# jzhoulab/orca

Hardware: AMD Instinct MI355X
Metric: Mb of sequence encoded+decoded per second (32Mb H1-ESC-shaped model, both strands, 6 levels) (higher is better)
Workload: dtype f16x2 | Encoder Conv1d stages 1-7: f16x2 = fp32 emulated as 2 x fp16 split operands, 3 MFMA products, fp32 accumulate (22 significant operand bits); Decoder / Decoder_1m Conv2d: f16x2 = fp32 emulated as 2 x fp16 split operands, 3 MFMA products, fp32 accumulate (22 significant operand bits); Encoder2; 1 GPU; H1-ESC 32Mb model forward, single random 32Mb sequence, fp32-class (f16x2 split operands on the 16-bit matrix cores, see dtype; parity vs the reference's fp32 in `parity` with --full), both strands (genomepredict-equivalent, 1 model): Encoder+Encoder2+6 Decoder+Decoder_1m per strand; sequence_bp=32000000, strands=2, levels=6, weights=synthetic seed 0, input=1 byte/base packed sequence in HBM, both strands read from it, parallelism=single GPU

## Files before the change

orca_amd/csrc/conv2d_dblock.h:

```cpp
#pragma once
#include "conv2d_m16.h"

struct DBlockArgs {
  f32x4* cur;
  const void* w[4];
  const float* bias[4];
  long bs;
  int H, W, dil;
  unsigned* flag;
};

#ifndef DBLOCK_STORE_WT
#define DBLOCK_STORE_WT 0
#endif
__device__ __forceinline__ void db_store_unit(u32x4_t* p, const u32x4_t& v) {
#if DBLOCK_STORE_WT
  m16_store_unit(p, v);
#else
  *p = v;
#endif
}

template <int NS, int DT, int ABL = 0>
__global__ __launch_bounds__(512, NS == 1 ? 4 : 2) void conv2d_dblock_kernel(DBlockArgs a) {
  constexpr int WNS = DT == 1 ? 2 : 1;
  constexpr int NT = 512, PXW = 256 + 16;
  constexpr int AU = NS * 8 * PXW, BU = NS * 4 * PXW;
  constexpr int WP = NS * 9 * 2 * 32;
  constexpr int NPIECE = 16;
  constexpr int WIT = (WP + NT - 1) / NT;
  static_assert(NS * 8 * 256 / NT == 4 * NS, "gather: NS DMA instructions per thread and K-chunk of the first layer (the same for every wave)");
  constexpr int EXTRA = (WP - (WIT - 1) * NT + 63) / 64;
  __shared__ f32x4 smem[AU + BU + 3 * WP + 48];
  f32x4* const As = smem;
  f32x4* const Bs = smem + AU;
  f32x4* const Ws = smem + AU + BU;
  float* const bias_s = reinterpret_cast<float*>(smem + AU + BU + 3 * WP);

  const int tid = threadIdx.x, lane = tid & 63;
  const int wave = __builtin_amdgcn_readfirstlane(tid >> 6);
  const int l31 = lane & 31, g = lane >> 5;
  const int d = a.dil, H = a.H, W = a.W;
  const int ld = 31 - __builtin_clz(d);
  const int lS = 8 - ld, S = 1 << lS;
  const int lG = 2 * ld - 8, G = 1 << lG;
  f32x4* const cur = a.cur + (long)blockIdx.y * a.bs;

  int bx = (int)blockIdx.x;
  if (!(ABL & 64)) {
    const int xcd = bx & 7, t = bx >> 3;
    if (G == 1) { const int run = xcd * 4 + (t >> 3); bx = (run >> 1) * 16 + (run & 1) * 8 + (t & 7); }
    else if (G == 4) { const int pair = xcd * 16 + (t >> 1); bx = pair * 2 + (t & 1); }
  }
  auto pix = [&](int p, int& row, int& col, int& r, int& c) {
    const int sid = (bx << lG) + (p >> (2 * lS)), q = p & ((1 << (2 * lS)) - 1);
    r = q >> lS; c = q & (S - 1);
    row = (sid >> ld) + (r << ld);
    col = (sid & (d - 1)) + (c << ld);
  };
  {
    const int sid0 = bx << lG;
    if ((sid0 >> ld) >= H || (sid0 & (d - 1)) >= W) return;
  }

  if (tid < NS * 8 * 16) As[(tid >> 4) * PXW + 256 + (tid & 15)] = (f32x4)(0.f);
  if (tid >= 256 && tid < 256 + NS * 4 * 16) Bs[((tid - 256) >> 4) * PXW + 256 + (tid & 15)] = (f32x4)(0.f);
  __syncthreads();
  if (wave == 0 && lane < 48) {
    const float* src = lane < 8 ? a.bias[0] + 4 * lane : (lane < 24 ? a.bias[1] + 4 * (lane - 8) : (lane < 32 ? a.bias[2] + 4 * (lane - 24) : a.bias[3] + 4 * (lane - 32)));
    p16_glds16(reinterpret_cast<const f32x4*>(src), smem + AU + BU + 3 * WP);
  }

  auto piece_src = [&](int i, int u) -> const f32x4* {
    const int L = i >> 2, j = i & 3;
    const bool wide = L & 1;
    const int k = wide ? (j & 1) : j, h = wide ? (j >> 1) : 0, cout = wide ? 64 : 32;
    const int grp = u >> 5, co = u & 31;
    return reinterpret_cast<const f32x4*>(a.w[L]) + ((long)k * (WNS * 9 * 2) + grp) * cout + h * 32 + co;
  };
  auto issue_piece = [&](int i) {
    f32x4* dst = Ws + (i % 3) * WP;
#pragma unroll
    for (int it = 0; it < WIT; ++it) {
      const int u = tid + it * NT;
      if (u < WP) p16_glds16(piece_src(i, u), dst + it * NT + wave * 64);
    }
  };
  {
    int row, col, r_, c_;
    pix(tid & 255, row, col, r_, c_);
    const bool ok = row < H && col < W;
    const long off = ok ? (long)row * M16_PX + col : 255;
#pragma unroll
    for (int k = 0; k < 4; ++k) {
#pragma unroll
      for (int s_ = 0; s_ < NS; ++s_) {
        const int plane = s_ * 8 + 2 * k + (wave >> 2);
        if (!(ABL & 4)) p16_glds16(cur + m16_plane(plane & 7, s_, NS, H) + off, As + plane * PXW + (wave & 3) * 64);
      }
      if (k < 3) issue_piece(k);
    }
  }

  const int p = wave * 32 + l31;
  int prow, pcol, pr, pc;
  pix(p, prow, pcol, pr, pc);
  const bool pvalid = prow < H && pcol < W;
  const long poff = (long)prow * M16_PX + pcol;
  unsigned nb16[9];
#pragma unroll
  for (int t = 0; t < 9; ++t) {
    const int dy = t / 3 - 1, dx = t % 3 - 1;
    const bool in = (unsigned)(pr + dy) < (unsigned)S && (unsigned)(pc + dx) < (unsigned)S;
    nb16[t] = (in ? (unsigned)(p + dy * S + dx) : 256u + ((unsigned)(p + dy * S + dx) & 15u)) * 16u;
  }

  f32x16 acc[2];
  int piece = 0;
  const unsigned as_lds = p16_lds_addr(As), bs_lds = p16_lds_addr(Bs), ws_lds = p16_lds_addr(Ws + g * 32 + l31);
#define DB_READ(buf_, t_)                                                                                         \
  _Pragma("unroll") for (int s = 0; s < NS; ++s) {                                                                \
    xv[buf_][s] = p16_lds_read16(xrow + nb16[t_], s * XG * PXW * 16);                                             \
    wv[buf_][s] = p16_lds_read16(wrow, ((s * 9 + (t_)) * 2) * 32 * 16);                                           \
  }
#define DB_LAYER(XLDS, XG_, WIDE)                                                                                 \
  {                                                                                                               \
    constexpr int XG = XG_;                                                                                       \
    _Pragma("unroll") for (int j = 0; j < 4; ++j, ++piece) {                                                      \
      constexpr bool wide_ = WIDE;                                                                                \
      const int k = wide_ ? (j & 1) : j;                                                                          \
      const int h = wide_ ? (j >> 1) : 0;                                                                         \
       \
       \
      if (piece == 0) {                                                                                           \
        if (wave < EXTRA) asm volatile("s_waitcnt vmcnt(%0)" ::"n"(3 * NS + 2 * WIT) : "memory");                \
        else asm volatile("s_waitcnt vmcnt(%0)" ::"n"(3 * NS + 2 * (WIT - 1)) : "memory");                       \
      } else if (piece == 1) {                                                                                    \
        if (wave < EXTRA) asm volatile("s_waitcnt vmcnt(%0)" ::"n"(2 * NS + WIT) : "memory");                    \
        else asm volatile("s_waitcnt vmcnt(%0)" ::"n"(2 * NS + WIT - 1) : "memory");                             \
      } else if (piece == 2) {                                                                                    \
        if (wave < EXTRA) asm volatile("s_waitcnt vmcnt(%0)" ::"n"(NS + WIT) : "memory");                        \
        else asm volatile("s_waitcnt vmcnt(%0)" ::"n"(NS + WIT - 1) : "memory");                                 \
      } else if (piece + 1 < NPIECE) {                                                                            \
        if (wave < EXTRA) asm volatile("s_waitcnt vmcnt(%0)" ::"n"(WIT) : "memory");                             \
        else asm volatile("s_waitcnt vmcnt(%0)" ::"n"(WIT - 1) : "memory");                                      \
      } else asm volatile("s_waitcnt vmcnt(0)" ::: "memory");                                                     \
       \
       \
       \
      if (!(ABL & 16) || j == 0) asm volatile("s_waitcnt lgkmcnt(0)\n\ts_barrier" ::: "memory");                                   \
      if (piece >= 1 && piece + 2 < NPIECE && !(ABL & 2)) issue_piece(piece + 2);    \
      const unsigned wrow = ws_lds + (unsigned)((piece % 3) * WP * 16);                                           \
      const unsigned xrow = (XLDS) + (unsigned)((2 * k + g) * PXW * 16);                                          \
      f16x8 xv[2][NS], wv[2][NS];                                                                                 \
      DB_READ(0, 0);                                                                                              \
      _Pragma("unroll") for (int t = 0; t < 9; ++t) {                                                             \
        const int fb = t & 1;                                                                                     \
        if (t + 1 < 9) { if (!(ABL & 8)) { DB_READ(fb ^ 1, t + 1); m16_wait<2 * NS, NS>(xv[fb], wv[fb]); } }      \
        else m16_wait<0, NS>(xv[fb], wv[fb]);                                                                     \
        typedef typename Op16<DT>::vec V_;                                                                        \
        if constexpr ((ABL & 1) != 0) { asm volatile("" ::"v"(xv[fb][0]), "v"(wv[fb][0])); } else                \
        if constexpr (NS == 2) {                                                                                  \
          acc[h] = Op16<DT>::mfma(__builtin_bit_cast(V_, wv[fb][0]), __builtin_bit_cast(V_, xv[fb][NS - 1]), acc[h]); \
          acc[h] = Op16<DT>::mfma(__builtin_bit_cast(V_, wv[fb][NS - 1]), __builtin_bit_cast(V_, xv[fb][0]), acc[h]); \
        }                                                                                                         \
        if constexpr ((ABL & 1) == 0) acc[h] = Op16<DT>::mfma(__builtin_bit_cast(V_, wv[fb][0]), __builtin_bit_cast(V_, xv[fb][0]), acc[h]); \
        __builtin_amdgcn_sched_barrier(0);                                                                        \
      }                                                                                                           \
    }                                                                                                             \
  }
  bool overflow = false;
  auto put = [&](f32x4* Xs, int XG, int oct, f32x4 v) {
    if (!pvalid) v = (f32x4)(0.f);
    u32x2 sp[NS];
    split4<NS, DT>(v, sp, overflow);
#pragma unroll
    for (int s = 0; s < NS; ++s) *reinterpret_cast<u32x2*>(reinterpret_cast<char*>(Xs + (s * XG + oct) * PXW + p) + 8 * g) = sp[s];
  };
  auto get_A = [&](int oct) -> f32x4 {
    float f[4] = {0.f, 0.f, 0.f, 0.f};
#pragma unroll
    for (int s = 0; s < NS; ++s) {
      const u32x2 u = *reinterpret_cast<const u32x2*>(reinterpret_cast<const char*>(As + (s * 8 + oct) * PXW + p) + 8 * g);
      float a0, a1, a2, a3;
      m16_pair<DT>(u.x, a0, a1);
      m16_pair<DT>(u.y, a2, a3);
      f[0] += a0; f[1] += a1; f[2] += a2; f[3] += a3;
    }
    f32x4 r;
    r.x = f[0]; r.y = f[1]; r.z = f[2]; r.w = f[3];
    return r;
  };
  auto acc4 = [&](int h, int q, int boff, bool relu) -> f32x4 {
    const f32x4 b = *reinterpret_cast<const f32x4*>(bias_s + boff + 8 * q + 4 * g);
    f32x4 v;
    v.x = acc[h][4 * q + 0] + b.x; v.y = acc[h][4 * q + 1] + b.y; v.z = acc[h][4 * q + 2] + b.z; v.w = acc[h][4 * q + 3] + b.w;
    if (relu) { v.x = p16_vmax(v.x, 0.f); v.y = p16_vmax(v.y, 0.f); v.z = p16_vmax(v.z, 0.f); v.w = p16_vmax(v.w, 0.f); }
    return v;
  };
  auto zero_acc = [&]() {
#pragma unroll
    for (int h = 0; h < 2; ++h)
#pragma unroll
      for (int r = 0; r < 16; ++r) acc[h][r] = 0.f;
  };

  zero_acc();
  DB_LAYER(as_lds, 8, false);
#pragma unroll
  for (int q = 0; q < 4; ++q) put(Bs, 4, q, acc4(0, q, 0, false));
  zero_acc();
  DB_LAYER(bs_lds, 4, true);
#pragma unroll
  for (int h = 0; h < 2; ++h)
#pragma unroll
    for (int q = 0; q < 4; ++q) put(As, 8, h * 4 + q, acc4(h, q, 32 + h * 32, false) + get_A(h * 4 + q));
  zero_acc();
  DB_LAYER(as_lds, 8, false);
#pragma unroll
  for (int q = 0; q < 4; ++q) put(Bs, 4, q, acc4(0, q, 96, true));
  zero_acc();
  DB_LAYER(bs_lds, 4, true);
#undef DB_LAYER
#undef DB_READ
  float vmax = 0.f;
  if constexpr (NS == 2) {
#pragma unroll
    for (int h = 0; h < 2; ++h)
#pragma unroll
      for (int q = 0; q < 4; ++q) {
        const f32x4 v = acc4(h, q, 128 + h * 32, true) + get_A(h * 4 + q);
        vmax = p16_vmax3_abs(p16_vmax3_abs(vmax, v.x, v.y), v.z, v.w);
        unsigned h0_, h1_, l0_, l1_;
        p16_split_hl(v, h0_, h1_, l0_, l1_);
        p16_swap32(h0_, l0_);
        p16_swap32(h1_, l1_);
        u32x4_t unit_;
        unit_.x = h0_; unit_.y = h1_; unit_.z = l0_; unit_.w = l1_;
        if (pvalid) db_store_unit(reinterpret_cast<u32x4_t*>(cur) + m16_plane(h * 4 + q, g, NS, H) + poff, unit_);
      }
    if (pvalid && vmax > 65504.f) overflow = true;
  } else {
#pragma unroll
    for (int h = 0; h < 2; ++h)
#pragma unroll
      for (int qp = 0; qp < 2; ++qp) {
        const f32x4 v0 = acc4(h, 2 * qp, 128 + h * 32, true) + get_A(h * 4 + 2 * qp);
        const f32x4 v1 = acc4(h, 2 * qp + 1, 128 + h * 32, true) + get_A(h * 4 + 2 * qp + 1);
        if (DT == 1) vmax = p16_vmax3_abs(p16_vmax3_abs(p16_vmax3_abs(p16_vmax3_abs(vmax, v0.x, v0.y), v0.z, v0.w), v1.x, v1.y), v1.z, v1.w);
        unsigned a0_ = m16_pk2<DT>(v0.x, v0.y), a1_ = m16_pk2<DT>(v0.z, v0.w), b0_ = m16_pk2<DT>(v1.x, v1.y), b1_ = m16_pk2<DT>(v1.z, v1.w);
        p16_swap32(a0_, b0_);
        p16_swap32(a1_, b1_);
        u32x4_t unit_;
        unit_.x = a0_; unit_.y = a1_; unit_.z = b0_; unit_.w = b1_;
        if (pvalid) db_store_unit(reinterpret_cast<u32x4_t*>(cur) + m16_plane(h * 4 + 2 * qp + g, 0, NS, H) + poff, unit_);
      }
    if (DT == 1 && pvalid && vmax > 65504.f) overflow = true;
  }
  if (DT == 1 && overflow && a.flag) *a.flag = 1u;
}
```

orca_amd/csrc/orca_decoder.hip:

```cpp
#include "orca_internal.h"

#include "conv2d_m16.h"
#include "conv2d_m16q.h"
#include "conv2d_dblock.h"
#include "misc_kernels.h"
#include "coarsegrain.h"

int launch_conv2d(orca_ctx* ctx, const ConvLayer& L, const float* x, long x_bs, float* y, long y_bs,
                         const float* r, long r_bs, int B, int n, int relu) {
  if (L.ksize != 3) return fail(ORCA_EINVAL, "launch_conv2d on a non-3x3 layer");
  Conv2dArgs a;
  a.x = x; a.w = L.d_w; a.bias = L.d_bias; a.y = y; a.r = r;
  a.x_bs = x_bs; a.y_bs = y_bs; a.r_bs = r_bs; a.H = n; a.W = n; a.dil = L.dil; a.nchunks = L.nchunks; a.relu = relu;
  dim3 grid((unsigned)n, (unsigned)B);
  if (L.cout == 64) hipLaunchKernelGGL((conv2d_3x3_kernel<64>), grid, dim3(512), 0, ctx->stream, a);
  else hipLaunchKernelGGL((conv2d_3x3_kernel<32>), grid, dim3(512), 0, ctx->stream, a);
  LAUNCHCHECK("conv2d_3x3_kernel");
  return ORCA_OK;
}

int launch_conv2d_m16(orca_ctx* ctx, const ConvLayer& L, const f32x4* x, long x_bs, int x_oct, f32x4* y, long y_bs, int y_oct,
                             const f32x4* r, long r_bs, int B, int n, int relu, int mode, int chunk0, int nchunks_,
                             const float* tab, long tab_bs) {
  const bool bf16 = mode == 1;
// ... 88 lines not shown
  ORCA_TRY(ws_ensure(ctx, need));
  auto take = [&](size_t units) { return reinterpret_cast<f32x4*>(ws_take(ctx, units * 4)); };
  float* const TAB0 = is1m ? nullptr : ws_take(ctx, B * tabsz);
  f32x4* const IN0 = take(B * szIN);
  f32x4* const A0 = take(B * szA);
  f32x4* const Bf0 = take(B * sz64);
  f32x4* const Cf0 = take(B * sz64);
  f32x4* const Df0 = take(B * sz64);
  f32x4* const T0 = take(B * sz32);
  auto run = [&](int b0, int nb) -> int {
    f32x4* IN = IN0 + b0 * szIN;
    f32x4* A = A0 + b0 * szA;
    f32x4* Bf = Bf0 + b0 * sz64;
    f32x4* Cf = Cf0 + b0 * sz64;
    f32x4* Df = Df0 + b0 * sz64;
    f32x4* T = T0 + b0 * sz32;
    hipStream_t s = ctx->stream;
    float* TAB = is1m ? nullptr : TAB0 + b0 * tabsz;
    auto emit = [&](const f32x4* buf, size_t bs) -> int {
      for (int b = 0; b < nb; ++b)
        hipLaunchKernelGGL((m16_to_nchw_kernel<NS, DT>), dim3((unsigned)n), dim3(ORCA_LDW), 0, s, buf + b * bs, probe->channels, n,
                           probe->out + (size_t)(b0 + b) * probe->channels * n * n);
      LAUNCHCHECK("m16_to_nchw_kernel");
      return ORCA_OK;
    };
#define PROBE(k, buf, bs) \
  if (probe && probe->stage == (k)) return emit(buf, bs)
    for (int c0 = 0; c0 < nb; c0 += 8) {
      const int nc = nb - c0 < 8 ? nb - c0 : 8;
      M16HeadArgs ha{};
      for (int b = 0; b < nc; ++b) { ha.x[b] = x.at(b0 + c0 + b); ha.de[b] = de.at(b0 + c0 + b); ha.y[b] = (!is1m && y) ? y.at(b0 + c0 + b) : nullptr; }
      ha.sx_c = sx_c; ha.sx_l = sx_l; ha.sd_c = sd_c; ha.sd_h = sd_h; ha.sd_w = sd_w; ha.sy_c = sy_c; ha.sy_h = sy_h; ha.sy_w = sy_w;
      ha.in = IN + c0 * szIN; ha.in_bs = (long)szIN;
      ha.tab = is1m ? nullptr : TAB + c0 * tabsz; ha.tab_bs = (long)tabsz;
      ha.a = A + c0 * szA; ha.a_bs = (long)szA;
      ha.wsep = net->d_sep; ha.nt = nt2; ha.n = n; ha.o0 = is1m ? 0 : 16; ha.noct = oIN; ha.nsep = is1m ? 0 : 6;
      ha.bilinear = net->upsample_mode == ORCA_UPSAMPLE_BILINEAR ? 1 : 0; ha.flag = ctx->d_flag;
      const unsigned roles = (unsigned)(oIN + ha.nsep + ((!is1m && y) ? 1 : 0));
      hipLaunchKernelGGL((decoder_head_m16_kernel<NS, DT>), dim3((unsigned)n, roles, (unsigned)nc), dim3(256), 0, s, ha);
      LAUNCHCHECK("decoder_head_m16_kernel");
    }
    PROBE(0, IN, szIN);
    const ConvLayer* L = net->convs.data();
    const ConvLayer* pairs;
    int npairs;
#define C2(layer, src, sbs, so, dst, dbs, dso, res, rbs, relu) \
  ORCA_TRY(launch_conv2d_m16(ctx, layer, src, sbs, so, dst, dbs, dso, res, rbs, nb, n, relu, mode))
    if (!is1m) {
      ORCA_TRY(launch_conv2d_m16(ctx, L[0], IN, szIN, oIN, Bf, sz64, 8, nullptr, 0, nb, n, 0, mode, 8, 1, TAB, (long)tabsz));
      PROBE(1, Bf, sz64);
      C2(L[1], Bf, sz64, 8, Cf, sz64, 8, nullptr, 0, 0);
      C2(L[2], Cf, sz64, 8, Bf, sz64, 8, nullptr, 0, 1);
      C2(L[3], Bf, sz64, 8, A, szA, oA, Cf, sz64, 1);
      PROBE(2, A, szA);
      pairs = L + 8; npairs = 28;
      if (y) {
        C2(L[4], A, szA, oA, Bf, sz64, 8, nullptr, 0, 0);
        C2(L[5], Bf, sz64, 8, Cf, sz64, 8, nullptr, 0, 0);
        C2(L[6], Cf, sz64, 8, Bf, sz64, 8, nullptr, 0, 1);
        C2(L[7], Bf, sz64, 8, Df, sz64, 8, Cf, sz64, 1);
      } else {
        C2(pairs[0], A, szA, oA, T, sz32, 4, nullptr, 0, 0);
        C2(pairs[1], T, sz32, 4, Cf, sz64, 8, nullptr, 0, 0);
        C2(pairs[2], Cf, sz64, 8, T, sz32, 4, nullptr, 0, 1);
        C2(pairs[3], T, sz32, 4, Df, sz64, 8, Cf, sz64, 1);
      }
    } else {
      pairs = L; npairs = 19;
      C2(pairs[0], IN, szIN, oIN, T, sz32, 4, nullptr, 0, 0);
      C2(pairs[1], T, sz32, 4, Cf, sz64, 8, nullptr, 0, 0);
      C2(pairs[2], Cf, sz64, 8, T, sz32, 4, nullptr, 0, 1);
      C2(pairs[3], T, sz32, 4, Df, sz64, 8, Cf, sz64, 1);
    }
    f32x4* cur = Df;
    f32x4* oth = Cf;
    for (int i = 1; i < npairs; ++i) {
      PROBE(3 + i - 1, cur, sz64);
      const ConvLayer* p = pairs + 4 * i;
      const int dil = p[0].dil;
      if (dil >= 16) {
        if (!(dil == 16 || dil == 32 || dil == 64) || p[1].dil != dil || p[2].dil != dil || p[3].dil != dil)
          return fail(ORCA_EINVAL, "decoder block %d: dilation %d unsupported", i, dil);
        DBlockArgs da;
        da.cur = cur; da.bs = sz64; da.H = n; da.W = n; da.dil = dil; da.flag = ctx->d_flag;
        for (int k = 0; k < 4; ++k) {
          if (!bf16 && !p[k].f16_ok) return fail(ORCA_EINVAL, "layer weights exceed the fp16 range");
          da.w[k] = bf16 ? p[k].d_wb16p : p[k].d_wf16;
          da.bias[k] = p[k].d_bias;
        }
        hipLaunchKernelGGL((conv2d_dblock_kernel<NS, DT>), dim3(256, (unsigned)nb), dim3(512), 0, ctx->stream, da);
        LAUNCHCHECK("conv2d_dblock_kernel");
        continue;
      }
      C2(p[0], cur, sz64, 8, T, sz32, 4, nullptr, 0, 0);
      C2(p[1], T, sz32, 4, oth, sz64, 8, cur, sz64, 0);
      C2(p[2], oth, sz64, 8, T, sz32, 4, nullptr, 0, 1);
      C2(p[3], T, sz32, 4, cur, sz64, 8, oth, sz64, 1);
    }
#undef C2
    PROBE(3 + npairs - 1, cur, sz64);
#undef PROBE
    const ConvLayer& fa = net->convs[net->convs.size() - 2];
    const ConvLayer& fb = net->convs[net->convs.size() - 1];
    FinalArgs fa_;
    fa_.cur = reinterpret_cast<const float*>(cur); fa_.w1 = fa.d_w; fa_.b1 = fa.d_bias; fa_.w2 = fb.d_w; fa_.b2 = fb.d_bias; fa_.out = out + (size_t)b0 * nt2 * n * n;
    fa_.cur_bs = sz64; fa_.out_bs = (long)nt2 * n * n; fa_.n = n; fa_.accumulate = accumulate; fa_.T = nt2; fa_.F = fa.cout;
    hipLaunchKernelGGL((final_sym_m16_kernel<NS, DT>), dim3(136u, (unsigned)nb), dim3(256), 0, s, fa_);
    LAUNCHCHECK("final_sym_m16_kernel");
    return ORCA_OK;
  };
  return run(0, B);
}

static int decoder_common(orca_ctx* ctx, orca_net* net, const RowSrc& x, long sx_c, long sx_l, const RowSrc& de,
                          long sd_c, long sd_h, long sd_w, const RowSrc& y, long sy_c, long sy_h, long sy_w,
                          int B, int n, float* out, int accumulate, const DecoderProbe* probe = nullptr) {
  const int nt2 = net->num_2d;
  if (n <= 0 || n > ORCA_LDW || (n & 1)) return fail(ORCA_EINVAL, "map size %d unsupported (even, <=256)", n);
  if (B <= 0) return ORCA_OK;
  HIPCHECK(hipSetDevice(ctx->device));
  if (net->precision == ORCA_PRECISION_F16X2)
    return decoder_m16<2, 1>(ctx, net, x, sx_c, sx_l, de, sd_c, sd_h, sd_w, y, sy_c, sy_h, sy_w, B, n, out, accumulate, probe);
  if (net->precision == ORCA_PRECISION_BF16)
    return decoder_m16<1, 0>(ctx, net, x, sx_c, sx_l, de, sd_c, sd_h, sd_w, y, sy_c, sy_h, sy_w, B, n, out, accumulate, probe);
  if (net->precision == ORCA_PRECISION_F16)
    return decoder_m16<1, 1>(ctx, net, x, sx_c, sx_l, de, sd_c, sd_h, sd_w, y, sy_c, sy_h, sy_w, B, n, out, accumulate, probe);
  if (probe) return fail(ORCA_EINVAL, "orca_decoder_probe: an f32 net has no M16 stages (its convs are conv2d_3x3_kernel)");
  const bool is1m = net->kind == ORCA_NET_DECODER_1M;
  const size_t plane = (size_t)n * ORCA_LDW;
  const int cin0 = is1m ? 128 : 136;
  const size_t szIN = plane * cin0, szA = plane * 72, sz64 = plane * 64, sz32 = plane * 32;
  const size_t need = ru256(B * szIN * 4) + ru256(B * szA * 4) + 3 * ru256(B * sz64 * 4) + ru256(B * sz32 * 4);
  ORCA_TRY(ws_ensure(ctx, need));
  float* IN = ws_take(ctx, B * szIN);
  float* A = ws_take(ctx, B * szA);
  float* Bf = ws_take(ctx, B * sz64);
  float* Cf = ws_take(ctx, B * sz64);
  float* Df = ws_take(ctx, B * sz64);
  float* T = ws_take(ctx, B * sz32);
  hipStream_t s = ctx->stream;
  for (int b = 0; b < B; ++b) {
    hipLaunchKernelGGL(outer_sum_kernel, dim3((unsigned)n, (unsigned)cin0), dim3(64), 0, s, x.at(b), sx_c, sx_l,
                       de.at(b), sd_c, sd_h, sd_w, nt2, IN + b * szIN, n, cin0);
    LAUNCHCHECK("outer_sum_kernel");
  }
  const ConvLayer* L = net->convs.data();
  const ConvLayer* pairs;
  int npairs;
  if (!is1m) {
    ORCA_TRY(launch_conv2d(ctx, L[0], IN, szIN, Bf, sz64, nullptr, 0, B, n, 0));
    ORCA_TRY(launch_conv2d(ctx, L[1], Bf, sz64, Cf, sz64, nullptr, 0, B, n, 0));
    ORCA_TRY(launch_conv2d(ctx, L[2], Cf, sz64, Bf, sz64, nullptr, 0, B, n, 1));
    ORCA_TRY(launch_conv2d(ctx, L[3], Bf, sz64, A, szA, Cf, sz64, B, n, 1));
    pairs = L + 8; npairs = 28;
    if (y) {
      for (int b = 0; b < B; ++b) {
        hipLaunchKernelGGL(upsample2d_x2_kernel, dim3((unsigned)n, 8), dim3(ORCA_LDW), 0, s, y.at(b), sy_c, sy_h, sy_w, nt2,
                           A + b * szA + 64 * plane, n, net->upsample_mode == ORCA_UPSAMPLE_BILINEAR ? 1 : 0, 8);
        LAUNCHCHECK("upsample2d_x2_kernel");
      }
      ORCA_TRY(launch_conv2d(ctx, L[4], A, szA, Bf, sz64, nullptr, 0, B, n, 0));
      ORCA_TRY(launch_conv2d(ctx, L[5], Bf, sz64, Cf, sz64, nullptr, 0, B, n, 0));
      ORCA_TRY(launch_conv2d(ctx, L[6], Cf, sz64, Bf, sz64, nullptr, 0, B, n, 1));
      ORCA_TRY(launch_conv2d(ctx, L[7], Bf, sz64, Df, sz64, Cf, sz64, B, n, 1));
    } else {
      ORCA_TRY(launch_conv2d(ctx, pairs[0], A, szA, T, sz32, nullptr, 0, B, n, 0));
      ORCA_TRY(launch_conv2d(ctx, pairs[1], T, sz32, Cf, sz64, nullptr, 0, B, n, 0));
      ORCA_TRY(launch_conv2d(ctx, pairs[2], Cf, sz64, T, sz32, nullptr, 0, B, n, 1));
      ORCA_TRY(launch_conv2d(ctx, pairs[3], T, sz32, Df, sz64, Cf, sz64, B, n, 1));
    }
  } else {
    pairs = L; npairs = 19;
    ORCA_TRY(launch_conv2d(ctx, pairs[0], IN, szIN, T, sz32, nullptr, 0, B, n, 0));
// ... 150 lines not shown
```

orca_amd/csrc/orca_test_entries.hip:

```cpp
#include "orca_internal.h"

#include "conv_p16.h"
#include "conv2d_m16.h"
#include "conv2d_dblock.h"
#include "misc_kernels.h"

extern "C" int orca_conv1d_forward(orca_ctx* ctx, const orca_conv_desc* conv, const float* x, int64_t x_bs, int64_t ldx, float* y,
                                   int64_t y_bs, int64_t ldy, const float* r1, const float* r2, int B, int64_t n, int relu,
                                   int tile) {
  if (!ctx || !conv || !x || !y) return fail(ORCA_EINVAL, "orca_conv1d_forward: NULL argument");
  HIPCHECK(hipSetDevice(ctx->device));
  ConvLayer L;
  ORCA_TRY(make_layer(*conv, &L));
  int rc = launch_conv1d(ctx, L, x, x_bs, ldx, y, y_bs, ldy, r1, r2, B, n, relu, tile);
  (void)hipStreamSynchronize(ctx->stream);
  free_layer(L);
  return rc;
}

extern "C" int orca_conv1d_nlc_forward(orca_ctx* ctx, const orca_conv_desc* conv, int precision, const float* x, float* y,
                                       const float* r1, int B, int64_t n, int relu) {
  if (!ctx || !conv || !x || !y) return fail(ORCA_EINVAL, "orca_conv1d_nlc_forward: NULL argument");
  if (precision < ORCA_PRECISION_BF16 || precision > ORCA_PRECISION_F16X2) return fail(ORCA_EINVAL, "precision %d unsupported here", precision);
  HIPCHECK(hipSetDevice(ctx->device));
// ... 59 lines not shown
                                       int relu, int out_mode) {
  if (conv && conv->cin % 32) return fail(ORCA_EINVAL, "orca_conv1d_b16_forward: cin %d is not a multiple of 32", conv->cin);
  return conv1d_planar_test(ctx, conv, x, y, r1, n, relu, out_mode, 1);
}

extern "C" int orca_conv2d_forward(orca_ctx* ctx, const orca_conv_desc* conv, const float* x, float* y, const float* r, int B,
                                   int n, int relu) {
  if (!ctx || !conv || !x || !y) return fail(ORCA_EINVAL, "orca_conv2d_forward: NULL argument");
  if (n <= 0 || n > ORCA_LDW) return fail(ORCA_EINVAL, "map size %d unsupported", n);
  HIPCHECK(hipSetDevice(ctx->device));
  ConvLayer L;
  ORCA_TRY(make_layer(*conv, &L));
  const int cpad = L.nchunks * 8;
  const size_t plane = (size_t)n * ORCA_LDW;
  int rc = ws_ensure(ctx, ru256(B * plane * cpad * 4) + 2 * ru256(B * plane * L.cout * 4));
  if (rc == ORCA_OK) {
    float* xp = ws_take(ctx, B * plane * cpad);
    float* yp = ws_take(ctx, B * plane * L.cout);
    float* rp = ws_take(ctx, B * plane * L.cout);
    hipStream_t s = ctx->stream;
    (void)hipMemsetAsync(xp, 0, B * plane * cpad * 4, s);
    for (int b = 0; b < B; ++b)
      hipLaunchKernelGGL(pad_rows_kernel, dim3((unsigned)(conv->cin * n)), dim3(ORCA_LDW), 0, s, x + (size_t)b * conv->cin * n * n,
                         xp + b * plane * cpad, n, 1);
    if (r) hipLaunchKernelGGL(pad_rows_kernel, dim3((unsigned)(B * L.cout * n)), dim3(ORCA_LDW), 0, s, r, rp, n, 1);
    rc = launch_conv2d(ctx, L, xp, plane * cpad, yp, plane * L.cout, r ? rp : nullptr, plane * L.cout, B, n, relu);
    if (rc == ORCA_OK) {
      hipLaunchKernelGGL(pad_rows_kernel, dim3((unsigned)(B * L.cout * n)), dim3(ORCA_LDW), 0, s, yp, y, n, 0);
      hipError_t e = hipGetLastError();
      if (e != hipSuccess) rc = fail(ORCA_EHIP, "pad_rows_kernel: %s", hipGetErrorString(e));
    }
  }
  (void)hipStreamSynchronize(ctx->stream);
  free_layer(L);
  return rc;
}

template <int NS, int DT>
static int conv2d_m16_test(orca_ctx* ctx, const ConvLayer& L, int mode, const float* x, float* y, const float* r, int B, int n, int relu) {
  const int xo = 2 * ((L.cin + 15) / 16), yo = L.cout / 8;
  const size_t upo = (size_t)NS * n * ORCA_LDW;
  ORCA_TRY(ws_ensure(ctx, ru256(B * upo * xo * 16) + 2 * ru256(B * upo * yo * 16)));
  f32x4* xp = reinterpret_cast<f32x4*>(ws_take(ctx, B * upo * xo * 4));
  f32x4* yp = reinterpret_cast<f32x4*>(ws_take(ctx, B * upo * yo * 4));
  f32x4* rp = reinterpret_cast<f32x4*>(ws_take(ctx, B * upo * yo * 4));
  hipStream_t s = ctx->stream;
  for (int b = 0; b < B; ++b) {
    hipLaunchKernelGGL((nchw_to_m16_kernel<NS, DT>), dim3((unsigned)n), dim3(ORCA_LDW), 0, s, x + (size_t)b * L.cin * n * n, L.cin, n, xp + b * upo * xo, xo);
    if (r) hipLaunchKernelGGL((nchw_to_m16_kernel<NS, DT>), dim3((unsigned)n), dim3(ORCA_LDW), 0, s, r + (size_t)b * L.cout * n * n, L.cout, n, rp + b * upo * yo, yo);
  }
  ORCA_TRY(launch_conv2d_m16(ctx, L, xp, upo * xo, xo, yp, upo * yo, yo, r ? rp : nullptr, upo * yo, B, n, relu, mode));
  for (int b = 0; b < B; ++b)
    hipLaunchKernelGGL((m16_to_nchw_kernel<NS, DT>), dim3((unsigned)n), dim3(ORCA_LDW), 0, s, yp + b * upo * yo, L.cout, n, y + (size_t)b * L.cout * n * n);
  LAUNCHCHECK("conv2d_m16 test path");
  return ORCA_OK;
}

extern "C" int orca_conv2d_m16_forward(orca_ctx* ctx, const orca_conv_desc* conv, int precision, const float* x, float* y, const float* r,
                                       int B, int n, int relu) {
  if (!ctx || !conv || !x || !y) return fail(ORCA_EINVAL, "orca_conv2d_m16_forward: NULL argument");
  if (n <= 0 || n > ORCA_LDW) return fail(ORCA_EINVAL, "map size %d unsupported", n);
  HIPCHECK(hipSetDevice(ctx->device));
  ConvLayer L;
  ORCA_TRY(make_layer(*conv, &L));
  int rc;
  if (precision == ORCA_PRECISION_F16X2) rc = conv2d_m16_test<2, 1>(ctx, L, 0, x, y, r, B, n, relu);
  else if (precision == ORCA_PRECISION_BF16) rc = conv2d_m16_test<1, 0>(ctx, L, 1, x, y, r, B, n, relu);
  else if (precision == ORCA_PRECISION_F16) rc = conv2d_m16_test<1, 1>(ctx, L, 2, x, y, r, B, n, relu);
  else rc = fail(ORCA_EINVAL, "orca_conv2d_m16_forward: precision %d has no M16 kernel", precision);
  (void)hipStreamSynchronize(ctx->stream);
  free_layer(L);
  return rc;
}

template <int NS, int DT>
static int conv2d_dblock_test(orca_ctx* ctx, const ConvLayer* L, const float* x, float* y, int B, int n) {
  const size_t sz64 = (size_t)NS * n * ORCA_LDW * 8;
  ORCA_TRY(ws_ensure(ctx, ru256(B * sz64 * 16)));
  f32x4* cur = reinterpret_cast<f32x4*>(ws_take(ctx, B * sz64 * 4));
  hipStream_t s = ctx->stream;
  for (int b = 0; b < B; ++b)
    hipLaunchKernelGGL((nchw_to_m16_kernel<NS, DT>), dim3((unsigned)n), dim3(ORCA_LDW), 0, s, x + (size_t)b * 64 * n * n, 64, n, cur + b * sz64, 8);
  DBlockArgs da;
  da.cur = cur; da.bs = (long)sz64; da.H = n; da.W = n; da.dil = L[0].dil; da.flag = ctx->d_flag;
  for (int k = 0; k < 4; ++k) {
    da.w[k] = DT == 0 ? L[k].d_wb16p : L[k].d_wf16;
    da.bias[k] = L[k].d_bias;
  }
  hipLaunchKernelGGL((conv2d_dblock_kernel<NS, DT>), dim3(256, (unsigned)B), dim3(512), 0, s, da);
  for (int b = 0; b < B; ++b)
    hipLaunchKernelGGL((m16_to_nchw_kernel<NS, DT>), dim3((unsigned)n), dim3(ORCA_LDW), 0, s, cur + b * sz64, 64, n, y + (size_t)b * 64 * n * n);
  LAUNCHCHECK("conv2d_dblock test path");
  return ORCA_OK;
}

extern "C" int orca_conv2d_dblock_forward(orca_ctx* ctx, const orca_conv_desc* convs, int precision, const float* x, float* y, int B, int n) {
  if (!ctx || !convs || !x || !y) return fail(ORCA_EINVAL, "orca_conv2d_dblock_forward: NULL argument");
  if (n <= 0 || n > ORCA_LDW || B <= 0 || B > 65535) return fail(ORCA_EINVAL, "orca_conv2d_dblock_forward: map size %d / batch %d unsupported", n, B);
  if (precision != ORCA_PRECISION_F16X2 && precision != ORCA_PRECISION_BF16 && precision != ORCA_PRECISION_F16)
    return fail(ORCA_EINVAL, "orca_conv2d_dblock_forward: precision %d has no block kernel", precision);
  const int d = convs[0].dilation;
  if (!(d == 16 || d == 32 || d == 64)) return fail(ORCA_EINVAL, "orca_conv2d_dblock_forward: dilation %d (16, 32 or 64)", d);
  for (int k = 0; k < 4; ++k) {
    const int cin = k & 1 ? 32 : 64, cout = k & 1 ? 64 : 32;
    if (convs[k].ksize != 3 || convs[k].cin != cin || convs[k].cout != cout || convs[k].dilation != d)
      return fail(ORCA_EINVAL, "orca_conv2d_dblock_forward: conv %d must be 3x3, %d -> %d, dilation %d", k, cin, cout, d);
  }
  HIPCHECK(hipSetDevice(ctx->device));
  ConvLayer L[4];
  int rc = ORCA_OK;
  for (int k = 0; k < 4 && rc == ORCA_OK; ++k) {
    rc = make_layer(convs[k], &L[k]);
    if (rc == ORCA_OK && precision != ORCA_PRECISION_BF16 && !L[k].f16_ok) rc = fail(ORCA_EINVAL, "layer weights exceed the fp16 range");
  }
  if (rc == ORCA_OK) {
    if (precision == ORCA_PRECISION_F16X2) rc = conv2d_dblock_test<2, 1>(ctx, L, x, y, B, n);
    else if (precision == ORCA_PRECISION_BF16) rc = conv2d_dblock_test<1, 0>(ctx, L, x, y, B, n);
    else rc = conv2d_dblock_test<1, 1>(ctx, L, x, y, B, n);
  }
  (void)hipStreamSynchronize(ctx->stream);
  for (int k = 0; k < 4; ++k) free_layer(L[k]);
  return rc;
}

extern "C" int orca_pointwise1d_forward(orca_ctx* ctx, const float* w_dev, const float* bias_dev, int cout, int cin, const float* x,
                                        int64_t x_bs, int64_t ldx, float* y, int64_t y_bs, int64_t ldy, int B, int64_t n, int act) {
  if (!ctx || !w_dev || !bias_dev || !x || !y) return fail(ORCA_EINVAL, "orca_pointwise1d_forward: NULL argument");
  if (cout <= 0 || cin <= 0 || B <= 0 || n < 0 || act < 0 || act > 2) return fail(ORCA_EINVAL, "orca_pointwise1d_forward: bad shape / activation");
  if (n == 0) return ORCA_OK;
  HIPCHECK(hipSetDevice(ctx->device));
  dim3 grid((unsigned)((n + 255) / 256), (unsigned)cout, (unsigned)B);
  hipLaunchKernelGGL(pointwise1d_kernel, grid, dim3(256), 0, ctx->stream, w_dev, bias_dev, cin, x, (long)x_bs, (long)ldx, y, (long)y_bs,
                     (long)ldy, (long)n, act);
  LAUNCHCHECK("pointwise1d_kernel");
  return ORCA_OK;
}

extern "C" int orca_maxpool1d_forward(orca_ctx* ctx, const float* x, int64_t ldx, float* y, int64_t ldy, int64_t rows,
                                      int64_t n_out, int k) {
  if (!ctx || !x || !y) return fail(ORCA_EINVAL, "orca_maxpool1d_forward: NULL argument");
  HIPCHECK(hipSetDevice(ctx->device));
  return launch_pool(ctx, x, ldx, y, ldy, rows, n_out, k);
}
```

Baseline: 986.8 Mb/s.

## Make decoder block kernel persistent over batch with cross-map prefetch

For the f16x2 path (NS==2), the fused 4-conv decoder block kernel now loops over several batch maps per workgroup instead of one. The grid's y-dimension is shrunk so the number of active tiles roughly fills 256 blocks. While the last layer of one map is finishing, it prefetches the next map's input gather and first weight pieces, rotating the triple-buffered weight slots. The final layer is split into two halves so the first half can be stored early. This is meant to cut launch and tail idle time and to hide the startup gather latency. The cost is longer per-block runtime, fewer blocks in flight, and more complex vmcnt bookkeeping that is easy to get wrong.

```diff
diff --git a/orca_amd/csrc/conv2d_dblock.h b/orca_amd/csrc/conv2d_dblock.h
--- a/orca_amd/csrc/conv2d_dblock.h
+++ b/orca_amd/csrc/conv2d_dblock.h
@@ -8,7 +8,23 @@
   long bs;
   int H, W, dil;
   unsigned* flag;
+  int nb;
 };
+
+template <int NS>
+inline dim3 dblock_grid(int nb, int H, int W, int dil) {
+  int ld = 0;
+  while ((1 << ld) < dil) ++ld;
+  const int lG = 2 * ld - 8;
+  int active = 0;
+  for (int bx = 0; bx < 256; ++bx) {
+    const int sid0 = bx << lG;
+    active += (sid0 >> ld) < H && (sid0 & (dil - 1)) < W;
+  }
+  int r = 256 / (active > 0 ? active : 1);
+  r = NS == 1 || r > nb ? nb : r;
+  return dim3(256, (unsigned)r);
+}
 
 #ifndef DBLOCK_STORE_WT
 #define DBLOCK_STORE_WT 0
@@ -28,6 +44,7 @@
   constexpr int AU = NS * 8 * PXW, BU = NS * 4 * PXW;
   constexpr int WP = NS * 9 * 2 * 32;
   constexpr int NPIECE = 16;
+  constexpr bool WALK = NS == 2;
   constexpr int WIT = (WP + NT - 1) / NT;
   static_assert(NS * 8 * 256 / NT == 4 * NS, "gather: NS DMA instructions per thread and K-chunk of the first layer (the same for every wave)");
   constexpr int EXTRA = (WP - (WIT - 1) * NT + 63) / 64;
@@ -37,14 +54,17 @@
   f32x4* const Ws = smem + AU + BU;
   float* const bias_s = reinterpret_cast<float*>(smem + AU + BU + 3 * WP);
 
-  const int tid = threadIdx.x, lane = tid & 63;
+  int tid = threadIdx.x;
+  const int lane = tid & 63;
   const int wave = __builtin_amdgcn_readfirstlane(tid >> 6);
-  const int l31 = lane & 31, g = lane >> 5;
+  int l31 = lane & 31, g = lane >> 5;
   const int d = a.dil, H = a.H, W = a.W;
   const int ld = 31 - __builtin_clz(d);
   const int lS = 8 - ld, S = 1 << lS;
   const int lG = 2 * ld - 8, G = 1 << lG;
-  f32x4* const cur = a.cur + (long)blockIdx.y * a.bs;
+  const int nb = a.nb, bstep = (int)gridDim.y;
+  int b = (int)blockIdx.y;
+  f32x4* cur = a.cur + (long)b * a.bs;
 
   int bx = (int)blockIdx.x;
   if (!(ABL & 64)) {
@@ -78,35 +98,40 @@
     const int grp = u >> 5, co = u & 31;
     return reinterpret_cast<const f32x4*>(a.w[L]) + ((long)k * (WNS * 9 * 2) + grp) * cout + h * 32 + co;
   };
+  int rb = 0;
+  auto slot = [&](int i) { const int s_ = i % 3 + rb; return s_ >= 3 ? s_ - 3 : s_; };
   auto issue_piece = [&](int i) {
-    f32x4* dst = Ws + (i % 3) * WP;
+    f32x4* dst = Ws + slot(i) * WP;
 #pragma unroll
     for (int it = 0; it < WIT; ++it) {
       const int u = tid + it * NT;
-      if (u < WP) p16_glds16(piece_src(i, u), dst + it * NT + wave * 64);
-    }
-  };
+      if (u < WP) p16_glds16(piece_src(i & 15, u), dst + it * NT + wave * 64);
+    }
+  };
+  int goff;
   {
     int row, col, r_, c_;
     pix(tid & 255, row, col, r_, c_);
-    const bool ok = row < H && col < W;
-    const long off = ok ? (long)row * M16_PX + col : 255;
-#pragma unroll
-    for (int k = 0; k < 4; ++k) {
-#pragma unroll
-      for (int s_ = 0; s_ < NS; ++s_) {
-        const int plane = s_ * 8 + 2 * k + (wave >> 2);
-        if (!(ABL & 4)) p16_glds16(cur + m16_plane(plane & 7, s_, NS, H) + off, As + plane * PXW + (wave & 3) * 64);
-      }
-      if (k < 3) issue_piece(k);
-    }
-  }
-
-  const int p = wave * 32 + l31;
+    goff = row < H && col < W ? row * M16_PX + col : 255;
+  }
+  auto issue_gather = [&](const f32x4* map, int k) {
+#pragma unroll
+    for (int s_ = 0; s_ < NS; ++s_) {
+      const int plane = s_ * 8 + 2 * k + (wave >> 2);
+      if (!(ABL & 4)) p16_glds16(map + m16_plane(plane & 7, s_, NS, H) + goff, As + plane * PXW + (wave & 3) * 64);
+    }
+  };
+#pragma unroll
+  for (int k = 0; k < 4; ++k) {
+    issue_gather(cur, k);
+    if (k < 3) issue_piece(k);
+  }
+
+  int p = wave * 32 + l31;
   int prow, pcol, pr, pc;
   pix(p, prow, pcol, pr, pc);
   const bool pvalid = prow < H && pcol < W;
-  const long poff = (long)prow * M16_PX + pcol;
+  int poff = prow * M16_PX + pcol;
   unsigned nb16[9];
 #pragma unroll
   for (int t = 0; t < 9; ++t) {
@@ -117,24 +142,42 @@
 
   f32x16 acc[2];
   int piece = 0;
-  const unsigned as_lds = p16_lds_addr(As), bs_lds = p16_lds_addr(Bs), ws_lds = p16_lds_addr(Ws + g * 32 + l31);
+  bool first = true;
+  bool more = WALK && b + bstep < nb;
+  f32x4* nxt = cur + (long)bstep * a.bs;
+  const unsigned as_lds = p16_lds_addr(As), bs_lds = p16_lds_addr(Bs);
+  unsigned ws_lds = p16_lds_addr(Ws + g * 32 + l31);
 #define DB_READ(buf_, t_)                                                                                         \
   _Pragma("unroll") for (int s = 0; s < NS; ++s) {                                                                \
     xv[buf_][s] = p16_lds_read16(xrow + nb16[t_], s * XG * PXW * 16);                                             \
     wv[buf_][s] = p16_lds_read16(wrow, ((s * 9 + (t_)) * 2) * 32 * 16);                                           \
   }
-#define DB_LAYER(XLDS, XG_, WIDE)                                                                                 \
+#define DB_LAYER(XLDS, XG_, WIDE, J0, J1)                                                                         \
   {                                                                                                               \
     constexpr int XG = XG_;                                                                                       \
-    _Pragma("unroll") for (int j = 0; j < 4; ++j, ++piece) {                                                      \
+    _Pragma("unroll") for (int j = J0; j < J1; ++j, ++piece) {                                                    \
       constexpr bool wide_ = WIDE;                                                                                \
       const int k = wide_ ? (j & 1) : j;                                                                          \
       const int h = wide_ ? (j >> 1) : 0;                                                                         \
        \
        \
+       \
+       \
+       \
+       \
+       \
+       \
+       \
+       \
+       \
       if (piece == 0) {                                                                                           \
-        if (wave < EXTRA) asm volatile("s_waitcnt vmcnt(%0)" ::"n"(3 * NS + 2 * WIT) : "memory");                \
-        else asm volatile("s_waitcnt vmcnt(%0)" ::"n"(3 * NS + 2 * (WIT - 1)) : "memory");                       \
+        if (first) {                                                                                              \
+          if (wave < EXTRA) asm volatile("s_waitcnt vmcnt(%0)" ::"n"(3 * NS + 2 * WIT) : "memory");              \
+          else asm volatile("s_waitcnt vmcnt(%0)" ::"n"(3 * NS + 2 * (WIT - 1)) : "memory");                     \
+        } else {                                                                                                  \
+          if (wave < EXTRA) asm volatile("s_waitcnt vmcnt(%0)" ::"n"(NS + WIT) : "memory");                      \
+          else asm volatile("s_waitcnt vmcnt(%0)" ::"n"(NS + WIT - 1) : "memory");                               \
+        }                                                                                                         \
       } else if (piece == 1) {                                                                                    \
         if (wave < EXTRA) asm volatile("s_waitcnt vmcnt(%0)" ::"n"(2 * NS + WIT) : "memory");                    \
         else asm volatile("s_waitcnt vmcnt(%0)" ::"n"(2 * NS + WIT - 1) : "memory");                             \
@@ -144,13 +187,23 @@
       } else if (piece + 1 < NPIECE) {                                                                            \
         if (wave < EXTRA) asm volatile("s_waitcnt vmcnt(%0)" ::"n"(WIT) : "memory");                             \
         else asm volatile("s_waitcnt vmcnt(%0)" ::"n"(WIT - 1) : "memory");                                      \
+      } else if (more) {                                                                                          \
+        if (wave < EXTRA) asm volatile("s_waitcnt vmcnt(%0)" ::"n"(2 * NS + WIT) : "memory");                    \
+        else asm volatile("s_waitcnt vmcnt(%0)" ::"n"(2 * NS + WIT - 1) : "memory");                             \
       } else asm volatile("s_waitcnt vmcnt(0)" ::: "memory");                                                     \
        \
        \
        \
       if (!(ABL & 16) || j == 0) asm volatile("s_waitcnt lgkmcnt(0)\n\ts_barrier" ::: "memory");                                   \
       if (piece >= 1 && piece + 2 < NPIECE && !(ABL & 2)) issue_piece(piece + 2);    \
-      const unsigned wrow = ws_lds + (unsigned)((piece % 3) * WP * 16);                                           \
+       \
+       \
+       \
+       \
+      if (piece == 14 && more) { issue_gather(nxt, 0); if (!(ABL & 2)) issue_piece(16); issue_gather(nxt, 1); }   \
+      if (piece == 15 && more && !(ABL & 2)) issue_piece(17);                                                     \
+      if (piece == 0 && !first) { issue_gather(cur, 2); if (!(ABL & 2)) issue_piece(2); issue_gather(cur, 3); }   \
+      const unsigned wrow = ws_lds + (unsigned)(slot(piece) * WP * 16);                                                 \
       const unsigned xrow = (XLDS) + (unsigned)((2 * k + g) * PXW * 16);                                          \
       f16x8 xv[2][NS], wv[2][NS];                                                                                 \
       DB_READ(0, 0);                                                                                              \
@@ -205,28 +258,9 @@
       for (int r = 0; r < 16; ++r) acc[h][r] = 0.f;
   };
 
-  zero_acc();
-  DB_LAYER(as_lds, 8, false);
-#pragma unroll
-  for (int q = 0; q < 4; ++q) put(Bs, 4, q, acc4(0, q, 0, false));
-  zero_acc();
-  DB_LAYER(bs_lds, 4, true);
-#pragma unroll
-  for (int h = 0; h < 2; ++h)
-#pragma unroll
-    for (int q = 0; q < 4; ++q) put(As, 8, h * 4 + q, acc4(h, q, 32 + h * 32, false) + get_A(h * 4 + q));
-  zero_acc();
-  DB_LAYER(as_lds, 8, false);
-#pragma unroll
-  for (int q = 0; q < 4; ++q) put(Bs, 4, q, acc4(0, q, 96, true));
-  zero_acc();
-  DB_LAYER(bs_lds, 4, true);
-#undef DB_LAYER
-#undef DB_READ
   float vmax = 0.f;
-  if constexpr (NS == 2) {
-#pragma unroll
-    for (int h = 0; h < 2; ++h)
+  auto store_half = [&](int h) {
+    if constexpr (NS == 2) {
 #pragma unroll
       for (int q = 0; q < 4; ++q) {
         const f32x4 v = acc4(h, q, 128 + h * 32, true) + get_A(h * 4 + q);
@@ -239,10 +273,7 @@
         unit_.x = h0_; unit_.y = h1_; unit_.z = l0_; unit_.w = l1_;
         if (pvalid) db_store_unit(reinterpret_cast<u32x4_t*>(cur) + m16_plane(h * 4 + q, g, NS, H) + poff, unit_);
       }
-    if (pvalid && vmax > 65504.f) overflow = true;
-  } else {
-#pragma unroll
-    for (int h = 0; h < 2; ++h)
+    } else {
 #pragma unroll
       for (int qp = 0; qp < 2; ++qp) {
         const f32x4 v0 = acc4(h, 2 * qp, 128 + h * 32, true) + get_A(h * 4 + 2 * qp);
@@ -255,7 +286,42 @@
         unit_.x = a0_; unit_.y = a1_; unit_.z = b0_; unit_.w = b1_;
         if (pvalid) db_store_unit(reinterpret_cast<u32x4_t*>(cur) + m16_plane(h * 4 + 2 * qp + g, 0, NS, H) + poff, unit_);
       }
-    if (DT == 1 && pvalid && vmax > 65504.f) overflow = true;
-  }
+    }
+  };
+
+  for (;;) {
+    piece = 0;
+    if constexpr (WALK) {
+      asm volatile("" : "+v"(tid), "+v"(p), "+v"(g), "+v"(poff), "+v"(ws_lds));
+#pragma unroll
+      for (int t = 0; t < 9; ++t) asm volatile("" : "+v"(nb16[t]));
+    }
+    zero_acc();
+    DB_LAYER(as_lds, 8, false, 0, 4);
+#pragma unroll
+    for (int q = 0; q < 4; ++q) put(Bs, 4, q, acc4(0, q, 0, false));
+    zero_acc();
+    DB_LAYER(bs_lds, 4, true, 0, 4);
+#pragma unroll
+    for (int h = 0; h < 2; ++h)
+#pragma unroll
+      for (int q = 0; q < 4; ++q) put(As, 8, h * 4 + q, acc4(h, q, 32 + h * 32, false) + get_A(h * 4 + q));
+    zero_acc();
+    DB_LAYER(as_lds, 8, false, 0, 4);
+#pragma unroll
+    for (int q = 0; q < 4; ++q) put(Bs, 4, q, acc4(0, q, 96, true));
+    zero_acc();
+    DB_LAYER(bs_lds, 4, true, 0, 2);
+    store_half(0);
+    DB_LAYER(bs_lds, 4, true, 2, 4);
+    store_half(1);
+    if (!WALK || !more) break;
+    b += bstep; cur = nxt; nxt = cur + (long)bstep * a.bs;
+    more = b + bstep < nb; first = false;
+    rb = rb == 2 ? 0 : rb + 1;
+  }
+#undef DB_LAYER
+#undef DB_READ
+  if (DT == 1 && pvalid && vmax > 65504.f) overflow = true;
   if (DT == 1 && overflow && a.flag) *a.flag = 1u;
 }
diff --git a/orca_amd/csrc/orca_decoder.hip b/orca_amd/csrc/orca_decoder.hip
--- a/orca_amd/csrc/orca_decoder.hip
+++ b/orca_amd/csrc/orca_decoder.hip
@@ -194,13 +194,13 @@
         if (!(dil == 16 || dil == 32 || dil == 64) || p[1].dil != dil || p[2].dil != dil || p[3].dil != dil)
           return fail(ORCA_EINVAL, "decoder block %d: dilation %d unsupported", i, dil);
         DBlockArgs da;
-        da.cur = cur; da.bs = sz64; da.H = n; da.W = n; da.dil = dil; da.flag = ctx->d_flag;
+        da.cur = cur; da.bs = sz64; da.H = n; da.W = n; da.dil = dil; da.flag = ctx->d_flag; da.nb = nb;
         for (int k = 0; k < 4; ++k) {
           if (!bf16 && !p[k].f16_ok) return fail(ORCA_EINVAL, "layer weights exceed the fp16 range");
           da.w[k] = bf16 ? p[k].d_wb16p : p[k].d_wf16;
           da.bias[k] = p[k].d_bias;
         }
-        hipLaunchKernelGGL((conv2d_dblock_kernel<NS, DT>), dim3(256, (unsigned)nb), dim3(512), 0, ctx->stream, da);
+        hipLaunchKernelGGL((conv2d_dblock_kernel<NS, DT>), dblock_grid<NS>(nb, n, n, dil), dim3(512), 0, ctx->stream, da);
         LAUNCHCHECK("conv2d_dblock_kernel");
         continue;
       }
diff --git a/orca_amd/csrc/orca_test_entries.hip b/orca_amd/csrc/orca_test_entries.hip
--- a/orca_amd/csrc/orca_test_entries.hip
+++ b/orca_amd/csrc/orca_test_entries.hip
@@ -165,12 +165,12 @@
   for (int b = 0; b < B; ++b)
     hipLaunchKernelGGL((nchw_to_m16_kernel<NS, DT>), dim3((unsigned)n), dim3(ORCA_LDW), 0, s, x + (size_t)b * 64 * n * n, 64, n, cur + b * sz64, 8);
   DBlockArgs da;
-  da.cur = cur; da.bs = (long)sz64; da.H = n; da.W = n; da.dil = L[0].dil; da.flag = ctx->d_flag;
+  da.cur = cur; da.bs = (long)sz64; da.H = n; da.W = n; da.dil = L[0].dil; da.flag = ctx->d_flag; da.nb = B;
   for (int k = 0; k < 4; ++k) {
     da.w[k] = DT == 0 ? L[k].d_wb16p : L[k].d_wf16;
     da.bias[k] = L[k].d_bias;
   }
-  hipLaunchKernelGGL((conv2d_dblock_kernel<NS, DT>), dim3(256, (unsigned)B), dim3(512), 0, s, da);
+  hipLaunchKernelGGL((conv2d_dblock_kernel<NS, DT>), dblock_grid<NS>(B, n, n, L[0].dil), dim3(512), 0, s, da);
   for (int b = 0; b < B; ++b)
     hipLaunchKernelGGL((m16_to_nchw_kernel<NS, DT>), dim3((unsigned)n), dim3(ORCA_LDW), 0, s, cur + b * sz64, 64, n, y + (size_t)b * 64 * n * n);
   LAUNCHCHECK("conv2d_dblock test path");
```

Result: no change. 992.4 Mb/s, median of 6 (+0.6%).
